# ImIntheMiddle/VATL4Pose-WACV2024

Measured on AMD Instinct MI355X. Metric: frames/sec pose-infer+uncertainty, 256x192 17-kp, higher is better.
Workload: dtype f32; 1 GPU; SimpleBaseline-R50 256x192 inference + decode + local-peak + THC-L1, 1024-frame synthetic video per GPU; frames_per_gpu=1024, batch=1024, tracks=4, parallelism=frame-sharded x1

## Files before the change

### include/vatl_hip.h

```cpp
#ifndef VATL_HIP_H
#define VATL_HIP_H

#include <stdint.h>

#ifdef __cplusplus
extern "C" {
#endif

#define VATL_VERSION 100
#define VATL_EINVAL  (-1)
#define VATL_ELAUNCH (-2)

int         vatl_version(void);
const char* vatl_last_error(void);

int vatl_flop_meter_begin(void);
int vatl_flop_meter_end(double* direct_flops, double* winograd_flops, int64_t* direct_launches, int64_t* winograd_launches);
#define VATL_ROUTE_NAMES "igemm,igemm_bnbwd,igemm_dma,persistent_1x1,streamk,rows_1x1,bottleneck_chain,stem_pool,halo_3x3," \
                         "winograd,winograd_2h,winograd_bnbwd,winograd_persist,winograd_c32,wgrad,winograd_wgrad,winograd_wgrad_2h," \
                         "winograd_wgrad_table,winograd_f4,winograd_f4_bnbwd,gemm1x1_ring,winograd_deconv43"
int vatl_flop_meter_routes(int64_t* counts, int n);


int vatl_nchw_to_nhwc(const float* src, float* dst, int N, int C, int H, int W, int Cpad, void* stream);
int vatl_nhwc_to_nchw(const float* src, float* dst, int N, int C, int H, int W, void* stream);

int vatl_pack_conv_weight(const float* w_oihw, float* w_packed, int Cout, int Cin, int R, int S,
                          int CoutPad, int Spad, int CinPad, void* stream);
int vatl_pack_deconv4x4s2_weight(const float* w_iohw, float* w_packed, int Cin, int Cout, int CoutPad, void* stream);
int64_t vatl_stem_pool_weight_floats(void);
int vatl_pack_stem_pool_weight(const float* w_oihw, float* packed, void* stream);
int vatl_stem_pool_supported(int H, int W);
int vatl_stem7x7s2_pool_fwd(const float* x_nchw, const float* w_packed, const float* scale, const float* bias, float* y_nhwc,
                            int N, int H, int W, void* stream);
int64_t vatl_stem3_weight_floats(void);
// ... 230 lines not shown
int vatl_conv3x3_winograd_fwd(const float* x, const float* u, const float* scale, const float* bias, const float* residual, float* y,
                              int N, int H, int W, int Cin, int Cout, int relu, void* stream);
int vatl_winograd_last_route(void);
int64_t vatl_winograd_stats_row_blocks(int64_t N, int H, int W);
int vatl_conv3x3_winograd_fwd_stats(const float* x, const float* u, float* y, double* stats, int64_t* row_blocks_used, int N, int H, int W,
                                    int Cin, int Cout, void* stream);
int64_t vatl_winograd_deconv_weight_floats(int Cout, int Cin);
int vatl_pack_winograd_deconv_weight(const float* w, float* u, int Cout, int Cin, void* stream);
int vatl_deconv4x4s2_winograd_fwd(const float* x, const float* u, const float* scale, const float* bias, float* y, int N, int H, int W,
                                  int Cin, int Cout, int relu, void* stream);
int64_t vatl_winograd_deconv43_weight_floats(int Cout, int Cin);
int vatl_pack_winograd_deconv43_weight(const float* w, float* u, int Cout, int Cin, void* stream);
int vatl_deconv4x4s2_winograd43_supported(int N, int H, int W, int Cin, int Cout);
int vatl_deconv4x4s2_winograd43_fwd(const float* x, const float* u, const float* scale, const float* bias, float* y, int N, int H, int W,
                                    int Cin, int Cout, int relu, void* stream);
int64_t vatl_winograd_deconv_stats_row_blocks(int64_t N, int H, int W);
int vatl_deconv4x4s2_winograd_fwd_stats(const float* x, const float* u, float* y, double* stats, int64_t* row_blocks_used, int N, int H, int W,
                                        int Cin, int Cout, void* stream);
int64_t vatl_conv3x3_winograd_wgrad_workspace_floats(int Cout, int Cin, int64_t N, int H, int W);
int vatl_conv3x3_winograd_wgrad(const float* x, const float* dz, float* dw, float* workspace, int N, int H, int W, int Cin, int Cout, void* stream);
int64_t vatl_deconv4x4s2_winograd_wgrad_workspace_floats(int Cin, int Cout, int64_t N, int H, int W);
int vatl_deconv4x4s2_winograd_wgrad(const float* x, const float* dy, float* dw, float* workspace, int N, int H, int W, int Cin, int Cout,
                                    void* stream);
int64_t vatl_winograd_deconv_dgrad_weight_floats(int Cin, int Cout);
int vatl_pack_winograd_deconv_dgrad_weight(const float* w, float* u, int Cin, int Cout, void* stream);
int vatl_deconv4x4s2_winograd_dgrad(const float* dz, const float* u, const float* residual, float* dx, int N, int H, int W, int Cin, int Cout,
                                    void* stream);
int vatl_deconv4x4s2_winograd_dgrad_bnbwd(const float* dz, const float* u, const float* residual, float* dx, int N, int H, int W, int Cin,
                                          int Cout, const float* bn_z, const float* bn_mask_y, const float* bn_scale, const float* bn_bias,
                                          const float* bn_mean, const float* bn_invstd, double* stats, int64_t* row_blocks_used, void* stream);
// ... 12 lines not shown
```

### vatl4pose-wacv2024_amd/alphapose/models/hip_engine.py

```python
from __future__ import annotations

import time
import weakref

import torch
import torch.nn as nn

import vatl_hip as vh

MAX_CHUNK = 1024



WINOGRAD = True
ROWS_GEMM = True
ROWS_GEMM_K = (128, 256)
WINO_C32 = True
WINO_F4 = True
DECONV_43 = True


class _Conv:
    __slots__ = ("w", "u", "u32", "u4", "wsrc", "wino", "c32", "f4", "scale", "bias", "cout", "r", "s", "stride", "pad")

    def __init__(self, conv: nn.Conv2d, bn: nn.BatchNorm2d | None):
        assert conv.groups == 1 and conv.dilation == (1, 1)
        assert conv.stride[0] == conv.stride[1] and conv.padding[0] == conv.padding[1]
        self.w = vh.pack_conv_weight(conv.weight.detach())
        self.cout, _, self.r, self.s = conv.weight.shape
        self.stride, self.pad = conv.stride[0], conv.padding[0]
        self.u = self.u32 = self.u4 = None
        self.wino = WINOGRAD and (self.r, self.s, self.stride, self.pad) == (3, 3, 1, 1) and conv.in_channels % 16 == 0 and self.cout % 4 == 0
        self.c32 = self.wino and WINO_C32 and conv.in_channels == 32 and self.cout == 32
        self.f4 = self.wino and WINO_F4 and conv.in_channels >= 64 and conv.in_channels % 16 == 0 and self.cout % 64 == 0
        self.wsrc = conv.weight.detach() if self.wino else None
        cb = conv.bias.detach() if conv.bias is not None else None
        if bn is not None:
            self.scale, self.bias = vh.bn_fold(_d(bn.weight), _d(bn.bias), bn.running_mean, bn.running_var, bn.eps, cb)
        elif cb is not None:
            self.scale, self.bias = vh.bn_fold(None, None, None, None, 0.0, cb, channels=self.cout)
        else:
            self.scale = self.bias = None

    def __call__(self, x, relu, residual=None, out_nchw=False, out=None):
        if self.wino and not out_nchw and not vh.latency_mode():
            if self.c32 and vh.conv3x3_winograd_c32_supported(x.shape[0], x.shape[1], x.shape[2], 32, 32):
                if self.u32 is None:
                    self.u32 = vh.pack_winograd_c32_weight(self.wsrc)
                return vh.conv3x3_winograd_c32_fwd(x, self.u32, self.scale, self.bias, relu, residual=residual, out=out)
            if self.f4 and vh.conv3x3_winograd_f4_supported(x.shape[0], x.shape[1], x.shape[2], x.shape[3], self.cout):
                if self.u4 is None:
                    self.u4 = vh.pack_winograd_f4_weight(self.wsrc)
                return vh.conv3x3_winograd_f4_fwd(x, self.u4, self.scale, self.bias, self.cout, relu, residual=residual, out=out)
            if self.u is None:
                self.u = vh.pack_winograd_weight(self.wsrc)
            return vh.conv3x3_winograd_fwd(x, self.u, self.scale, self.bias, self.cout, relu, residual=residual, out=out)
        if (ROWS_GEMM and self.r == 1 and self.stride == 1 and not out_nchw and not vh.latency_mode() and x.shape[-1] in ROWS_GEMM_K
                and vh.conv1x1_rows_supported(x.shape[-1], 0, self.cout, x.shape[0] * x.shape[1] * x.shape[2])):
            return vh.conv1x1_rows_fwd(x, self.w, self.scale, self.bias, self.cout, relu, residual=residual, out=out)
        return vh.conv2d_fwd(x, self.w, self.scale, self.bias, self.cout, self.r, self.s, self.stride, self.pad, relu,
                             residual=residual, out_nchw=out_nchw, out=out)


class _Deconv:
    __slots__ = ("w", "u", "u43", "wsrc", "d43", "scale", "bias", "cout")

    def __init__(self, dc: nn.ConvTranspose2d, bn: nn.BatchNorm2d):
        assert dc.kernel_size == (4, 4) and dc.stride == (2, 2) and dc.padding == (1, 1) and dc.bias is None
        self.cout = dc.weight.shape[1]
        self.u = self.u43 = None
        self.d43 = WINOGRAD and DECONV_43 and dc.weight.shape[0] % 16 == 0 and self.cout % 64 == 0
        self.wsrc = dc.weight.detach() if self.d43 else None
        if WINOGRAD and dc.weight.shape[0] % 16 == 0 and self.cout % 4 == 0:
            self.u = vh.pack_winograd_deconv_weight(dc.weight.detach())
        self.w = vh.pack_deconv_weight(dc.weight.detach())
        self.scale, self.bias = vh.bn_fold(_d(bn.weight), _d(bn.bias), bn.running_mean, bn.running_var, bn.eps)
# ... 498 lines not shown
```

### vatl4pose-wacv2024_amd/csrc/common.h

```cpp
#pragma once
#include <hip/hip_runtime.h>
#include <atomic>
#include <cstdarg>
#include <cstdio>
#include <cstdint>

#include "vatl_hip.h"

namespace vatl {

char* err_buf();
int fail(int code, const char* fmt, ...);

void meter_add(int kind, double flops);
enum MeterRoute {
    kRouteIgemm = 0, kRouteIgemmBnBwd, kRouteIgemmDma, kRoutePersistent1x1, kRouteStreamK, kRouteRows, kRouteChain, kRouteStemPool, kRouteHalo,
    kRouteWino, kRouteWino2H, kRouteWinoBnBwd, kRouteWinoPersist, kRouteWinoC32, kRouteWgrad, kRouteWinoWgrad, kRouteWinoWgrad2H,
    kRouteWinoWgradTable, kRouteWinoF4, kRouteWinoF4BnBwd, kRouteGemm1x1Ring, kRouteWinoDeconv43, kRouteCount
};
void meter_route(int route);

inline int check_launch(const char* what) {
    hipError_t e = hipGetLastError();
    if (e != hipSuccess) return fail(VATL_ELAUNCH, "%s: %s", what, hipGetErrorString(e));
    return 0;
}

inline int ensure_dynamic_lds(const void* kern, int bytes, std::atomic<unsigned>& done_mask, const char* what) {
    int d = 0;
    if (hipGetDevice(&d) != hipSuccess) return fail(VATL_ELAUNCH, "%s: no current device", what);
    const unsigned bit = 1u << (d & 31);
    if (done_mask.load(std::memory_order_acquire) & bit) return 0;
    hipError_t e = hipFuncSetAttribute(kern, hipFuncAttributeMaxDynamicSharedMemorySize, bytes);
// ... 59 lines not shown
```

### vatl4pose-wacv2024_amd/csrc/pack.hip

```cpp
#include "glue_common.h"
#include "winograd_pack.h"

namespace vatl {

template <class I>
__device__ __forceinline__ float pack_conv_elem(const float* __restrict__ w, I i, int Cout, int Cin, int R, int S, int Spad, int CinPad) {
    const I c = i % (I)CinPad;
    I t = i / (I)CinPad;
    const I s = t % (I)Spad; t /= (I)Spad;
    const I r = t % (I)R;
    const I o = t / (I)R;
    float v = 0.f;
    if ((int)o < Cout && (int)s < S && (int)c < Cin) v = w[(((long long)o * Cin + c) * R + r) * S + s];
    return v;
}

template <class I>
__device__ __forceinline__ float pack_deconv_elem(const float* __restrict__ w, I i, int Cin, int Cout, int CoutPad) {
    const I c = i % (I)Cin;
    I t = i / (I)Cin;
    const int tx = (int)(t & 1); t >>= 1;
    const int ty = (int)(t & 1); t >>= 1;
    const I o = t % (I)CoutPad;
    const int ph = (int)(t / (I)CoutPad);
// ... 66 lines not shown
    if (c >= C) return;
    float s = 1.f, b = 0.f;
    if (var) {
        s = (gamma ? gamma[c] : 1.f) / sqrtf(var[c] + eps);
        b = (beta ? beta[c] : 0.f) - mean[c] * s;
    }
    if (cbias) b += cbias[c] * s;
    scale[c] = s;
    bias[c] = b;
}

__global__ __launch_bounds__(256) void wino43_pack_kernel(const float* __restrict__ w, float* __restrict__ out, int Cout, int Cin) {
    wino43_pack_block(w, out, Cout, Cin, blockIdx.x, threadIdx.x);
}

__global__ __launch_bounds__(256) void pack_multi_kernel(const VatlPackJob* __restrict__ jobs, int njobs) {
    __shared__ int sj;
    if (threadIdx.x == 0) {
        int lo = 0, hi = njobs - 1;
        const long long b = blockIdx.x;
        while (lo < hi) {
            const int mid = (lo + hi + 1) >> 1;
            if (jobs[mid].first_block <= b) lo = mid; else hi = mid - 1;
        }
        sj = lo;
    }
    __syncthreads();
    const VatlPackJob* J = jobs + sj;
    const float* __restrict__ w = J->src;
    float* __restrict__ out = J->dst;
// ... 47 lines not shown
    hipLaunchKernelGGL(pack_deconv_weight_kernel, dim3(ew_grid(16LL * CoutPad * Cin)), dim3(256), 0, (hipStream_t)stream, w, out, Cin, Cout, CoutPad);
    return check_launch("pack_deconv4x4s2_weight");
}

extern "C" int64_t vatl_winograd_deconv43_weight_floats(int Cout, int Cin) { return 4LL * 20 * Cout * Cin; }

extern "C" int vatl_pack_winograd_deconv43_weight(const float* w, float* u, int Cout, int Cin, void* stream) {
    if (!w || !u || Cout <= 0 || Cin <= 0) return fail(VATL_EINVAL, "pack_winograd_deconv43_weight: null pointer or empty filter");
    if (Cin % 16 != 0 || Cout % 64 != 0) return fail(VATL_EINVAL, "pack_winograd_deconv43_weight: Cin %d must be a multiple of 16 and Cout %d of 64", Cin, Cout);
    const long long blocks = 4LL * (Cout / 32) * (Cin / 8);
    if (blocks > 0x7FFFFFFF) return fail(VATL_EINVAL, "pack_winograd_deconv43_weight: filter too large");
    hipLaunchKernelGGL(wino43_pack_kernel, dim3((unsigned)blocks), dim3(256), 0, (hipStream_t)stream, w, u, Cout, Cin);
    return check_launch("wino43_pack");
}

extern "C" int vatl_pack_dgrad_weight(const float* w_oihw, float* out, int Cout, int Cin, int R, int S, int CinPad, int CoutK,
                                      int ntaps, const int* tap_r, const int* tap_s, void* stream) {
    if (!w_oihw || !out || !tap_r || !tap_s || ntaps < 1 || ntaps > 16 || CinPad < Cin || CoutK < Cout) return fail(VATL_EINVAL, "pack_dgrad_weight: bad arguments");
    TapList t{};
    t.n = ntaps;
    for (int i = 0; i < ntaps; ++i) {
        if (tap_r[i] < 0 || tap_r[i] >= R || tap_s[i] < 0 || tap_s[i] >= S) return fail(VATL_EINVAL, "pack_dgrad_weight: tap %d out of range", i);
        t.r[i] = tap_r[i]; t.s[i] = tap_s[i];
    }
    hipLaunchKernelGGL(pack_dgrad_weight_kernel, dim3((unsigned)((long long)cdiv(CinPad, 32) * ntaps * cdiv(CoutK, 32))), dim3(256), 0, (hipStream_t)stream,
                       w_oihw, out, Cout, Cin, R, S, CinPad, CoutK, t);
    return check_launch("pack_dgrad_weight");
}

extern "C" int vatl_pack_weights_multi(const VatlPackJob* jobs_device, int njobs, int64_t total_blocks, void* stream) {
// ... 13 lines not shown
```

### vatl4pose-wacv2024_amd/csrc/winograd_pack.h

```cpp
#pragma once

namespace vatl {

__device__ __forceinline__ void wino_pack_block(const float* __restrict__ w, float* __restrict__ out, int mode, int w_i, int Cout, int Cin, int NH,
                                                long long bl, int tid) {
    const int steps = Cin >> 3;
    int phase = 0;
    if (mode >= 2) {
        const long long per = (long long)((Cout + 32 * NH - 1) / (32 * NH)) * NH * steps;
        phase = (int)(bl / per);
        bl -= phase * per;
        out += phase * per * 4096;
    }
    const int n32 = (int)(bl / steps), step = (int)(bl - (long long)n32 * steps);
    const int nl = tid & 31, cc = tid >> 5;
    const int n = n32 * 32 + nl, c = step * 8 + cc;
    const int n_tile = n32 / NH, nh = n32 - n_tile * NH;
    const int lane = (cc >> 2) * 32 + nl, tt = cc & 3;
    double tg[4][3];
    if (mode >= 2) {
        const int py = phase >> 1, px = phase & 1;
        double g[2][2];
#pragma unroll
        for (int a = 0; a < 2; ++a)
// ... 59 lines not shown
        for (int b = 0; b < 2; ++b) g[a][b] = (double)w[(((long long)c * Cout + n) * 4 + (3 - py - 2 * a)) * 4 + (3 - px - 2 * b)];
    float* o = out + ((((long long)((n32 >> 1) * steps + step) * 20) * 2 + (n32 & 1)) * 64 + (cc >> 2) * 32 + nl) * 4 + (cc & 3);
#pragma unroll
    for (int xi = 0; xi < 5; ++xi)
#pragma unroll
        for (int nu = 0; nu < 4; ++nu) {
            double v = 0.0;
#pragma unroll
            for (int a = 0; a < 2; ++a)
#pragma unroll
                for (int b = 0; b < 2; ++b) v += G4[xi][a] * g[a][b] * G3[nu][b];
            o[(long long)(xi * 4 + nu) * 512] = (float)v;
        }
}

__device__ __forceinline__ void f4_pack_item(const float* __restrict__ w, float* __restrict__ u, int dgrad, int w_i, int Cout, int Cin, long long id) {
    const int nbg = Cout >> 4;
    const long long total = (long long)(Cin >> 4) * 36 * nbg * 64;
    if (id >= total) return;
    const int lane = (int)(id & 63);
    const int blk = (int)((id >> 6) % nbg);
    const int pos = (int)((id >> 6) / nbg % 36);
    const int stage = (int)((id >> 6) / nbg / 36);
    const int xi = pos / 6, nu = pos - 6 * xi;
    const double G[6][3] = {{0.25, 0, 0}, {-1.0 / 6, -1.0 / 6, -1.0 / 6}, {-1.0 / 6, 1.0 / 6, -1.0 / 6}, {1.0 / 24, 1.0 / 12, 1.0 / 6}, {1.0 / 24, -1.0 / 12, 1.0 / 6}, {0, 0, 1}};
    const int n = 16 * blk + (lane & 15);
    float o[4];
#pragma unroll
    for (int s = 0; s < 4; ++s) {
        const int c = 16 * stage + 4 * (lane >> 4) + s;
// ... 14 lines not shown
```

### vatl4pose-wacv2024_amd/vatl_hip/__init__.py

```python
from __future__ import annotations

import ctypes as C
import os
import threading as _threading

import torch

_HERE = os.path.dirname(os.path.abspath(__file__))
LIB_PATH = os.environ.get("VATL_HIP_LIB") or os.path.join(_HERE, "libvatl_hip.so")

_p = C.c_void_p
_i = C.c_int
_f = C.c_float
_d = C.c_double
_i64 = C.c_int64

SIGNATURES = {
    "vatl_version": (_i, []),
    "vatl_last_error": (C.c_char_p, []),
    "vatl_flop_meter_begin": (_i, []),
    "vatl_flop_meter_end": (_i, [_p, _p, _p, _p]),
    "vatl_flop_meter_routes": (_i, [_p, _i]),
    "vatl_nchw_to_nhwc": (_i, [_p, _p, _i, _i, _i, _i, _i, _p]),
    "vatl_nhwc_to_nchw": (_i, [_p, _p, _i, _i, _i, _i, _p]),
# ... 77 lines not shown
    "vatl_conv3x3_winograd_wgrad_workspace_floats": (_i64, [_i, _i, _i64, _i, _i]),
    "vatl_conv3x3_winograd_wgrad": (_i, [_p] * 4 + [_i] * 5 + [_p]),
    "vatl_deconv4x4s2_winograd_wgrad_workspace_floats": (_i64, [_i, _i, _i64, _i, _i]),
    "vatl_deconv4x4s2_winograd_wgrad": (_i, [_p] * 4 + [_i] * 5 + [_p]),
    "vatl_winograd_deconv_dgrad_weight_floats": (_i64, [_i, _i]),
    "vatl_pack_winograd_deconv_dgrad_weight": (_i, [_p, _p, _i, _i, _p]),
    "vatl_deconv4x4s2_winograd_dgrad": (_i, [_p] * 4 + [_i] * 5 + [_p]),
    "vatl_deconv4x4s2_winograd_dgrad_bnbwd": (_i, [_p] * 4 + [_i] * 5 + [_p] * 9),
    "vatl_winograd_deconv_weight_floats": (_i64, [_i, _i]),
    "vatl_pack_winograd_deconv_weight": (_i, [_p, _p, _i, _i, _p]),
    "vatl_deconv4x4s2_winograd_fwd": (_i, [_p] * 5 + [_i] * 6 + [_p]),
    "vatl_winograd_deconv43_weight_floats": (_i64, [_i, _i]),
    "vatl_pack_winograd_deconv43_weight": (_i, [_p, _p, _i, _i, _p]),
    "vatl_deconv4x4s2_winograd43_supported": (_i, [_i, _i, _i, _i, _i]),
    "vatl_deconv4x4s2_winograd43_fwd": (_i, [_p] * 5 + [_i] * 6 + [_p]),
    "vatl_winograd_deconv_stats_row_blocks": (_i64, [_i64, _i, _i]),
    "vatl_deconv4x4s2_winograd_fwd_stats": (_i, [_p, _p, _p, _p, _p, _i, _i, _i, _i, _i, _p]),
    "vatl_conv2d_fwd_stats": (_i, [_p, _p, _p, _p, _p, _i, _i, _i, _i, _i, _i, _i, _i, _i, _i, _p]),
    "vatl_deconv4x4s2_fwd_stats": (_i, [_p, _p, _p, _p, _p, _i, _i, _i, _i, _i, _i, _p]),
    "vatl_bn_train_finalize": (_i, [_p, _i64, _i64, _i, _p, _p, _p, _p, _f, _f, _p, _p, _p, _p, _p]),
    "vatl_maxpool3x3s2_bwd": (_i, [_p, _p, _p, _i, _i, _i, _i, _p]),
    "vatl_maxpool3x3s2_fwd_idx": (_i, [_p, _p, _p, _i, _i, _i, _i, _p]),
    "vatl_pack_weights_multi": (_i, [_p, _i, _i64, _p]),
    "vatl_adamw_multi_block_elems": (_i64, []),
    "vatl_checksum_block_words": (_i64, []),
    "vatl_checksum_multi": (_i, [_p, _i, _i64, _p, _p]),
    "vatl_maxpool3x3s2_fwd_idx_affine": (_i, [_p, _p, _p, _p, _p, _i, _i, _i, _i, _p]),
    "vatl_bn_train_bwd_relu_pool": (_i, [_p, _p, _p, _p, _p, _p, _p, _p, _p, _p, _p, _i, _i, _i, _i, _p, _p, _p]),
    "vatl_maxpool3x3s2_bwd_idx": (_i, [_p, _p, _p, _i, _i, _i, _i, _p]),
    "vatl_pixelunshuffle2": (_i, [_p, _p, _i, _i, _i, _i, _p]),
# ... 98 lines not shown
    y = torch.empty((n, h, w, cpad), device=x.device, dtype=torch.float32)
    _check(lib().vatl_nchw_to_nhwc(_ptr(x), _ptr(y), n, c, h, w, cpad, _stream()), "vatl_nchw_to_nhwc")
    return y


def nhwc_to_nchw(x: torch.Tensor) -> torch.Tensor:
    n, h, w, c = x.shape
    y = torch.empty((n, c, h, w), device=x.device, dtype=torch.float32)
    _check(lib().vatl_nhwc_to_nchw(_ptr(x), _ptr(y), n, c, h, w, _stream()), "vatl_nhwc_to_nchw")
    return y



ROUTE_NAMES = ("igemm", "igemm_bnbwd", "igemm_dma", "persistent_1x1", "streamk", "rows_1x1", "bottleneck_chain", "stem_pool", "halo_3x3", "winograd",
               "winograd_2h", "winograd_bnbwd", "winograd_persist", "winograd_c32", "wgrad", "winograd_wgrad", "winograd_wgrad_2h", "winograd_wgrad_table", "winograd_f4", "winograd_f4_bnbwd",
               "gemm1x1_ring", "winograd_deconv43")


class flop_meter:

    def __enter__(self):
        _check(lib().vatl_flop_meter_begin(), "flop_meter_begin")
        self.direct = self.winograd = self.total = 0.0
        self.direct_launches = self.winograd_launches = 0
        return self

    @staticmethod
    def launches_now() -> int:
        counts = (C.c_int64 * len(ROUTE_NAMES))()
        _check(min(0, lib().vatl_flop_meter_routes(counts, len(ROUTE_NAMES))), "flop_meter_routes")
        return int(sum(counts))
# ... 264 lines not shown
    if tuple(w.shape[2:]) != (4, 4):
        raise VatlError("pack_winograd_deconv_weight: 4x4 filters only")
    return _pack(("winograd_deconv", w.data_ptr(), tuple(w.shape)), w, lambda: (
        int(lib().vatl_winograd_deconv_weight_floats(cout, cin)), "vatl_pack_winograd_deconv_weight", (cout, cin),
        _winograd_fields(_PACK_WINOGRAD_DECONV, cout, cin, 4, cout)))


def pack_winograd_deconv43_weight(w: torch.Tensor) -> torch.Tensor:
    cin, cout = w.shape[:2]
    if tuple(w.shape[2:]) != (4, 4):
        raise VatlError("pack_winograd_deconv43_weight: 4x4 filters only")
    return _pack(("winograd_deconv43", w.data_ptr(), tuple(w.shape)), w, lambda: (
        int(lib().vatl_winograd_deconv43_weight_floats(cout, cin)), "vatl_pack_winograd_deconv43_weight", (cout, cin), None), planned=False)


def pack_winograd_deconv_dgrad_weight(w: torch.Tensor) -> torch.Tensor:
    cin, cout = w.shape[:2]
    if tuple(w.shape[2:]) != (4, 4):
        raise VatlError("pack_winograd_deconv_dgrad_weight: 4x4 filters only")
    return _pack(("winograd_deconv_dgrad", w.data_ptr(), tuple(w.shape)), w, lambda: (
        int(lib().vatl_winograd_deconv_dgrad_weight_floats(cin, cout)), "vatl_pack_winograd_deconv_dgrad_weight", (cin, cout),
        _winograd_fields(_PACK_WINOGRAD_DECONV_DGRAD, cin, cout, 4, cout)))


def pack_conv1x1_dual_weight(w1, scale1, bias1, w2, scale2, bias2):
    cout, c1 = w1.shape[:2]
    c2 = w2.shape[1]
    cpad = conv_cout_pad(cout)
    out = torch.empty((cpad, c1 + c2), device=w1.device, dtype=torch.float32)
    bias = torch.empty(cout, device=w1.device, dtype=torch.float32)
# ... 26 lines not shown
    out = torch.empty(int(lib().vatl_stem3_weight_floats()), device=w.device, dtype=torch.float32)
    _check(lib().vatl_pack_stem3_weight(_ptr(w), _ptr(out), _stream()), "vatl_pack_stem3_weight")
    return out


def bn_fold(gamma, beta, mean, var, eps: float, conv_bias=None, channels: int | None = None):
    c = channels if channels is not None else (var.numel() if var is not None else conv_bias.numel())
    dev = (var if var is not None else conv_bias).device
    scale = torch.empty(c, device=dev, dtype=torch.float32)
    bias = torch.empty(c, device=dev, dtype=torch.float32)
    _check(lib().vatl_bn_fold(_ptr(gamma), _ptr(beta), _ptr(mean), _ptr(var), _ptr(conv_bias), eps, _ptr(scale), _ptr(bias), c, _stream()), "vatl_bn_fold")
    return scale, bias



def conv2d_fwd(x, w_packed, scale, bias, cout: int, r: int, s: int, stride: int, pad: int, relu: bool,
               residual=None, out_nchw: bool = False, out=None):
    n, h, w, cin = x.shape
    ho = (h + 2 * pad - r) // stride + 1
    wo = (w + 2 * pad - s) // stride + 1
    shape = (n, cout, ho, wo) if out_nchw else (n, ho, wo, cout)
    y = out if out is not None else torch.empty(shape, device=x.device, dtype=torch.float32)
    _check(lib().vatl_conv2d_fwd(_ptr(x), _ptr(w_packed), _ptr(scale), _ptr(bias), _ptr(residual), _ptr(y), n, h, w, cin, cout,
                                 w_packed.shape[0], r, s, stride, pad, int(relu), int(out_nchw), _stream()), "vatl_conv2d_fwd")
    return y


def conv1x1_dual_fwd(a, x, w_packed, bias, cout: int, stride2: int, relu: bool, out=None):
    n, ho, wo, c1 = a.shape
    _, h2, w2, c2 = x.shape
    y = out if out is not None else torch.empty((n, ho, wo, cout), device=a.device, dtype=torch.float32)
    _check(lib().vatl_conv1x1_dual_fwd(_ptr(a), _ptr(x), _ptr(w_packed), _ptr(bias), _ptr(y), n, ho, wo, c1, h2, w2, c2, stride2, cout,
                                       w_packed.shape[0], int(relu), _stream()), "vatl_conv1x1_dual_fwd")
    return y


def conv1x1_rows_supported(k1: int, k2: int, n: int, m: int) -> bool:
# ... 879 lines not shown
```

Measured before the change: 17030 frames/s.

## Add polyphase Winograd F(4x4? ,3x3) kernel for stride-2 3x3 convolutions

Adds a new Winograd kernel for stride-2 3x3 convs. It splits the filter into four polyphase sub-filters (2x2 taps) and transforms each into a Winograd domain, producing 4x3 output tiles, with matching weight packing and buffer-load-to-LDS staging into MFMA accumulation. The ResNet-50 downsampling convs in layers 2-4 are routed to it when there is no residual, the output is NHWC, and the shape meets H%8 and W%6. This cuts multiply work compared with the direct implicit GEMM. In exchange it adds transform overhead and fp32 rounding differences, and it only applies to shapes that meet the divisibility constraints.

```diff
diff --git a/include/vatl_hip.h b/include/vatl_hip.h
--- a/include/vatl_hip.h
+++ b/include/vatl_hip.h
@@ -18,7 +18,7 @@
 int vatl_flop_meter_end(double* direct_flops, double* winograd_flops, int64_t* direct_launches, int64_t* winograd_launches);
 #define VATL_ROUTE_NAMES "igemm,igemm_bnbwd,igemm_dma,persistent_1x1,streamk,rows_1x1,bottleneck_chain,stem_pool,halo_3x3," \
                          "winograd,winograd_2h,winograd_bnbwd,winograd_persist,winograd_c32,wgrad,winograd_wgrad,winograd_wgrad_2h," \
-                         "winograd_wgrad_table,winograd_f4,winograd_f4_bnbwd,gemm1x1_ring,winograd_deconv43"
+                         "winograd_wgrad_table,winograd_f4,winograd_f4_bnbwd,gemm1x1_ring,winograd_deconv43,winograd_s2_43"
 int vatl_flop_meter_routes(int64_t* counts, int n);
 
 
@@ -279,6 +279,11 @@
 int vatl_deconv4x4s2_winograd43_supported(int N, int H, int W, int Cin, int Cout);
 int vatl_deconv4x4s2_winograd43_fwd(const float* x, const float* u, const float* scale, const float* bias, float* y, int N, int H, int W,
                                     int Cin, int Cout, int relu, void* stream);
+int64_t vatl_winograd_s2_43_weight_floats(int Cout, int Cin);
+int vatl_pack_winograd_s2_43_weight(const float* w, float* u, int Cout, int Cin, void* stream);
+int vatl_conv3x3s2_winograd43_supported(int N, int H, int W, int Cin, int Cout);
+int vatl_conv3x3s2_winograd43_fwd(const float* x, const float* u, const float* scale, const float* bias, float* y, int N, int H, int W,
+                                  int Cin, int Cout, int relu, void* stream);
 int64_t vatl_winograd_deconv_stats_row_blocks(int64_t N, int H, int W);
 int vatl_deconv4x4s2_winograd_fwd_stats(const float* x, const float* u, float* y, double* stats, int64_t* row_blocks_used, int N, int H, int W,
                                         int Cin, int Cout, void* stream);
diff --git a/vatl4pose-wacv2024_amd/alphapose/models/hip_engine.py b/vatl4pose-wacv2024_amd/alphapose/models/hip_engine.py
--- a/vatl4pose-wacv2024_amd/alphapose/models/hip_engine.py
+++ b/vatl4pose-wacv2024_amd/alphapose/models/hip_engine.py
@@ -18,10 +18,11 @@
 WINO_C32 = True
 WINO_F4 = True
 DECONV_43 = True
+S2_43 = True
 
 
 class _Conv:
-    __slots__ = ("w", "u", "u32", "u4", "wsrc", "wino", "c32", "f4", "scale", "bias", "cout", "r", "s", "stride", "pad")
+    __slots__ = ("w", "u", "u32", "u4", "us2", "wsrc", "wino", "c32", "f4", "s2", "scale", "bias", "cout", "r", "s", "stride", "pad")
 
     def __init__(self, conv: nn.Conv2d, bn: nn.BatchNorm2d | None):
         assert conv.groups == 1 and conv.dilation == (1, 1)
@@ -33,7 +34,9 @@
         self.wino = WINOGRAD and (self.r, self.s, self.stride, self.pad) == (3, 3, 1, 1) and conv.in_channels % 16 == 0 and self.cout % 4 == 0
         self.c32 = self.wino and WINO_C32 and conv.in_channels == 32 and self.cout == 32
         self.f4 = self.wino and WINO_F4 and conv.in_channels >= 64 and conv.in_channels % 16 == 0 and self.cout % 64 == 0
-        self.wsrc = conv.weight.detach() if self.wino else None
+        self.us2 = None
+        self.s2 = WINOGRAD and S2_43 and (self.r, self.s, self.stride, self.pad) == (3, 3, 2, 1) and conv.in_channels % 16 == 0 and self.cout % 64 == 0
+        self.wsrc = conv.weight.detach() if self.wino or self.s2 else None
         cb = conv.bias.detach() if conv.bias is not None else None
         if bn is not None:
             self.scale, self.bias = vh.bn_fold(_d(bn.weight), _d(bn.bias), bn.running_mean, bn.running_var, bn.eps, cb)
@@ -58,8 +61,13 @@
         if (ROWS_GEMM and self.r == 1 and self.stride == 1 and not out_nchw and not vh.latency_mode() and x.shape[-1] in ROWS_GEMM_K
                 and vh.conv1x1_rows_supported(x.shape[-1], 0, self.cout, x.shape[0] * x.shape[1] * x.shape[2])):
             return vh.conv1x1_rows_fwd(x, self.w, self.scale, self.bias, self.cout, relu, residual=residual, out=out)
+        us2 = None
+        if self.s2 and residual is None and not out_nchw and not vh.latency_mode():
+            if self.us2 is None and vh.conv3x3s2_winograd43_supported(x.shape[0], x.shape[1], x.shape[2], x.shape[3], self.cout):
+                self.us2 = vh.pack_winograd_s2_43_weight(self.wsrc)
+            us2 = self.us2
         return vh.conv2d_fwd(x, self.w, self.scale, self.bias, self.cout, self.r, self.s, self.stride, self.pad, relu,
-                             residual=residual, out_nchw=out_nchw, out=out)
+                             residual=residual, out_nchw=out_nchw, out=out, u_s2=us2)
 
 
 class _Deconv:
diff --git a/vatl4pose-wacv2024_amd/csrc/common.h b/vatl4pose-wacv2024_amd/csrc/common.h
--- a/vatl4pose-wacv2024_amd/csrc/common.h
+++ b/vatl4pose-wacv2024_amd/csrc/common.h
@@ -16,7 +16,7 @@
 enum MeterRoute {
     kRouteIgemm = 0, kRouteIgemmBnBwd, kRouteIgemmDma, kRoutePersistent1x1, kRouteStreamK, kRouteRows, kRouteChain, kRouteStemPool, kRouteHalo,
     kRouteWino, kRouteWino2H, kRouteWinoBnBwd, kRouteWinoPersist, kRouteWinoC32, kRouteWgrad, kRouteWinoWgrad, kRouteWinoWgrad2H,
-    kRouteWinoWgradTable, kRouteWinoF4, kRouteWinoF4BnBwd, kRouteGemm1x1Ring, kRouteWinoDeconv43, kRouteCount
+    kRouteWinoWgradTable, kRouteWinoF4, kRouteWinoF4BnBwd, kRouteGemm1x1Ring, kRouteWinoDeconv43, kRouteWinoS2_43, kRouteCount
 };
 void meter_route(int route);
 
diff --git a/vatl4pose-wacv2024_amd/csrc/pack.hip b/vatl4pose-wacv2024_amd/csrc/pack.hip
--- a/vatl4pose-wacv2024_amd/csrc/pack.hip
+++ b/vatl4pose-wacv2024_amd/csrc/pack.hip
@@ -104,6 +104,10 @@
     wino43_pack_block(w, out, Cout, Cin, blockIdx.x, threadIdx.x);
 }
 
+__global__ __launch_bounds__(256) void wino_s2_43_pack_kernel(const float* __restrict__ w, float* __restrict__ out, int Cout, int Cin) {
+    wino_s2_43_pack_block(w, out, Cout, Cin, blockIdx.x, threadIdx.x);
+}
+
 __global__ __launch_bounds__(256) void pack_multi_kernel(const VatlPackJob* __restrict__ jobs, int njobs) {
     __shared__ int sj;
     if (threadIdx.x == 0) {
@@ -181,6 +185,17 @@
     return check_launch("wino43_pack");
 }
 
+extern "C" int64_t vatl_winograd_s2_43_weight_floats(int Cout, int Cin) { return 72LL * Cout * Cin; }
+
+extern "C" int vatl_pack_winograd_s2_43_weight(const float* w, float* u, int Cout, int Cin, void* stream) {
+    if (!w || !u || Cout <= 0 || Cin <= 0) return fail(VATL_EINVAL, "pack_winograd_s2_43_weight: null pointer or empty filter");
+    if (Cin % 16 != 0 || Cout % 64 != 0) return fail(VATL_EINVAL, "pack_winograd_s2_43_weight: Cin %d must be a multiple of 16 and Cout %d of 64", Cin, Cout);
+    const long long blocks = 4LL * (Cout / 32) * (Cin / 8);
+    if (blocks > 0x7FFFFFFF) return fail(VATL_EINVAL, "pack_winograd_s2_43_weight: filter too large");
+    hipLaunchKernelGGL(wino_s2_43_pack_kernel, dim3((unsigned)blocks), dim3(256), 0, (hipStream_t)stream, w, u, Cout, Cin);
+    return check_launch("wino_s2_43_pack");
+}
+
 extern "C" int vatl_pack_dgrad_weight(const float* w_oihw, float* out, int Cout, int Cin, int R, int S, int CinPad, int CoutK,
                                       int ntaps, const int* tap_r, const int* tap_s, void* stream) {
     if (!w_oihw || !out || !tap_r || !tap_s || ntaps < 1 || ntaps > 16 || CinPad < Cin || CoutK < Cout) return fail(VATL_EINVAL, "pack_dgrad_weight: bad arguments");
diff --git a/vatl4pose-wacv2024_amd/csrc/winograd_pack.h b/vatl4pose-wacv2024_amd/csrc/winograd_pack.h
--- a/vatl4pose-wacv2024_amd/csrc/winograd_pack.h
+++ b/vatl4pose-wacv2024_amd/csrc/winograd_pack.h
@@ -97,6 +97,41 @@
         }
 }
 
+__device__ __forceinline__ void wino_s2_43_pack_block(const float* __restrict__ w, float* __restrict__ out, int Cout, int Cin, long long bl, int tid) {
+    const int steps = Cin >> 3;
+    const long long per = (long long)(Cout >> 5) * steps;
+    const int phase = (int)(bl / per);
+    bl -= phase * per;
+    const int n32 = (int)(bl / steps), step = (int)(bl - (long long)n32 * steps);
+    const int nl = tid & 31, cc = tid >> 5;
+    const int n = n32 * 32 + nl, c = step * 8 + cc;
+    const int by = phase >> 1, bx = phase & 1;
+    const double G4[5][2] = {{0.5, 0.0}, {-0.5, -0.5}, {-1.0 / 6, 1.0 / 6}, {1.0 / 6, 1.0 / 3}, {0.0, 1.0}};
+    const double G3[4][2] = {{1.0, 0.0}, {0.5, 0.5}, {0.5, -0.5}, {0.0, -1.0}};
+    double g[2][2];
+#pragma unroll
+    for (int a = 0; a < 2; ++a)
+#pragma unroll
+        for (int b = 0; b < 2; ++b)
+            g[a][b] = (2 * a + by < 3 && 2 * b + bx < 3) ? (double)w[(((long long)n * Cin + c) * 3 + (2 * a + by)) * 3 + (2 * b + bx)] : 0.0;
+    const long long gstep = (long long)bx * steps + step;
+    float* o = out + (long long)(n32 >> 1) * steps * 36864 + (by ? (long long)steps * 20480 + gstep * 8192 : gstep * 10240) +
+               ((n32 & 1) * 64 + (cc >> 2) * 32 + nl) * 4 + (cc & 3);
+#pragma unroll
+    for (int xi = 0; xi < 5; ++xi) {
+        if (by && xi == 4) continue;
+#pragma unroll
+        for (int nu = 0; nu < 4; ++nu) {
+            double v = 0.0;
+#pragma unroll
+            for (int a = 0; a < 2; ++a)
+#pragma unroll
+                for (int b = 0; b < 2; ++b) v += G4[xi][a] * g[a][b] * G3[nu][b];
+            o[(long long)(xi * 4 + nu) * 512] = (float)v;
+        }
+    }
+}
+
 __device__ __forceinline__ void f4_pack_item(const float* __restrict__ w, float* __restrict__ u, int dgrad, int w_i, int Cout, int Cin, long long id) {
     const int nbg = Cout >> 4;
     const long long total = (long long)(Cin >> 4) * 36 * nbg * 64;
diff --git a/vatl4pose-wacv2024_amd/csrc/winograd_s2_43.hip b/vatl4pose-wacv2024_amd/csrc/winograd_s2_43.hip
--- /dev/null
+++ b/vatl4pose-wacv2024_amd/csrc/winograd_s2_43.hip
@@ -0,0 +1,313 @@
+#include "common.h"
+#include "buffer.h"
+
+#include <algorithm>
+#include <atomic>
+#include <type_traits>
+
+namespace vatl {
+
+struct S2W43Params {
+    const float* x;
+    const float* u;
+    const float* scale;
+    const float* bias;
+    float* y;
+    int N, H, W, Cin, Cout;
+    int OH, OW;
+    int TH, TW, tpi, Mtiles;
+    int m_tiles, n_tiles;
+    int relu;
+    int sp;
+    int rn;
+    unsigned x_bytes, u_bytes, y_bytes;
+    FastDivU d_TH, d_TW, d_tpi, d_grp, d_rn, d_rn_last;
+};
+
+constexpr unsigned S2W_OOB = 0xFFFF0000u;
+constexpr int S2W_TB = 32;
+constexpr int S2W_CK = 16;
+constexpr int S2W_NQ = S2W_TB + 1;
+constexpr int S2W_ROWE = 3 * S2W_NQ + 1;
+constexpr int S2W_ROWF = S2W_ROWE * S2W_CK;
+constexpr int S2W_ITEMS = 5 * S2W_ROWE * 4;
+constexpr int S2W_NDMA = (S2W_ITEMS + 63) / 64;
+constexpr int S2W_ROW4_DMA = 4 * S2W_ROWE * 4 / 64;
+constexpr int S2W_STAGE = S2W_NDMA * 256;
+constexpr int S2W_NLD = S2W_NDMA / 4;
+constexpr int S2W_LDS_BYTES = 2 * S2W_STAGE * 4;
+static_assert(S2W_NDMA % 4 == 0 && 16 * S2W_TB * 32 * 4 == S2W_LDS_BYTES, "stage buffers = output-transform tiles");
+static_assert(4 * S2W_ROWE * 4 % 64 == 0, "the fifth input row starts a DMA instruction");
+
+__device__ __forceinline__ void winograd_s2_43_body(const S2W43Params& p, float* smem) {
+    constexpr int NW = 4;
+    float* Rs = smem;
+    const int tid = threadIdx.x, lane = tid & 63, nu = __builtin_amdgcn_readfirstlane(tid >> 6);
+
+    const int bid = blockIdx.x, nblk = gridDim.x;
+    const int xcd = bid & 7, loc = bid >> 3, q8 = nblk >> 3, r8 = nblk & 7;
+    const int t = (xcd < r8 ? xcd * (q8 + 1) : r8 * (q8 + 1) + (xcd - r8) * q8) + loc;
+    const int grp = fdiv(t, p.d_grp), rem = t - grp * (p.m_tiles * p.rn);
+    const bool last_grp = p.n_tiles - grp * p.rn < p.rn;
+    const int rn_g = last_grp ? p.n_tiles - grp * p.rn : p.rn;
+    const int m_tile = fdiv(rem, last_grp ? p.d_rn_last : p.d_rn), n_tile = grp * p.rn + (rem - m_tile * rn_g);
+    const int m0 = m_tile * S2W_TB, n0 = n_tile * 64;
+
+    const __amdgpu_buffer_rsrc_t xr = buf_rsrc(p.x, p.x_bytes);
+    const __amdgpu_buffer_rsrc_t ur = buf_rsrc(p.u, p.u_bytes);
+
+    const int steps = p.sp * 2;
+    const int gsteps = 4 * steps, gsteps5 = 2 * steps;
+    const unsigned ubase = (unsigned)n_tile * (unsigned)steps * 147456u + ((unsigned)((nu * 2) * 64 + lane) << 4);
+    auto u_load = [&](auto np, f32x4 (&dst)[5], int gstep_, int half) {
+        constexpr int NP = decltype(np)::value;
+        const int g = min(gstep_, gsteps - 1);
+        const unsigned soff = g < gsteps5 ? (unsigned)g * 40960u : (unsigned)gsteps5 * 40960u + (unsigned)(g - gsteps5) * 32768u;
+        const unsigned off = ubase + (unsigned)half * 1024u + soff;
+#pragma unroll
+        for (int xi = 0; xi < NP; ++xi) dst[xi] = buf_load4(ur, off + xi * 8192u);
+    };
+    f32x4 ua[5], ub[5];
+    u_load(std::integral_constant<int, 5>{}, ua, 0, 0);
+
+    unsigned goff[S2W_NLD];
+    auto set_goff = [&](int pad_y, int pad_x) {
+        int m0 = m_tile * S2W_TB, ln = lane;
+        asm volatile("" : "+s"(m0), "+v"(ln));
+#pragma unroll
+        for (int u = 0; u < S2W_NLD; ++u) {
+            __builtin_amdgcn_sched_barrier(0);
+            const int pz = (nu + NW * u) * 64 + ln;
+            goff[u] = S2W_OOB;
+            if (pz >= S2W_ITEMS) continue;
+            const int cpos = pz & 3, e = pz >> 2;
+            const int i = e / S2W_ROWE, re = e - i * S2W_ROWE;
+            const int r = re / S2W_NQ, q = re - r * S2W_NQ;
+            if (r >= 3) continue;
+            const int chunk = cpos ^ ((q >> 2) & 3);
+            int m = m0 + q;
+            int gr = fdiv(m, p.d_TW), tx = m - gr * p.TW;
+            int xx = 3 * tx + r - pad_x;
+            if (m >= p.Mtiles || (tx == 0 && xx < 0)) {
+                m -= 1;
+                if (m < 0) continue;
+                gr = fdiv(m, p.d_TW); tx = m - gr * p.TW;
+                xx = 3 * tx + 3 + r - pad_x;
+            }
+            const int b = fdiv(gr, p.d_TH), ty = gr - b * p.TH;
+            const int yy = 4 * ty - pad_y + i;
+            if (m < p.Mtiles && (unsigned)yy < (unsigned)p.OH && (unsigned)xx < (unsigned)p.OW)
+                goff[u] = (unsigned)(((b * p.H + 2 * yy + pad_y) * p.W + 2 * xx + pad_x) * p.Cin + chunk * 4) << 2;
+        }
+    };
+    auto stage_dma = [&](int buf, int st, bool rows5) {
+        unsigned so = (unsigned)st * (S2W_CK * 4);
+        asm volatile("" : "+s"(so));
+#pragma unroll
+        for (int u = 0; u < S2W_NLD; ++u) {
+            if (!rows5 && nu + NW * u >= S2W_ROW4_DMA) continue;
+            __builtin_amdgcn_raw_ptr_buffer_load_lds(xr, (lds_void*)(Rs + buf * S2W_STAGE + (nu + NW * u) * 256), 16,
+                                                     goff[u] + so, 0, 0, 0);
+        }
+    };
+    set_goff(1, 1);
+    stage_dma(0, 0, true);
+
+    const int ja = nu == 0 ? 0 : (nu == 2 ? 2 : 1);
+    const int jb = nu == 0 ? 2 : (nu == 1 ? 2 : (nu == 2 ? 1 : 3));
+    const float sgn = nu == 1 ? 1.f : -1.f;
+    int ca, cb;
+    auto set_cols = [&](int pad_x) {
+        int ln = lane;
+        asm volatile("" : "+v"(ln));
+        const int tl = ln & 31, h = ln >> 5;
+        const int m = min(m0 + tl, p.Mtiles - 1);
+        const int gr = fdiv(m, p.d_TW), tx = m - gr * p.TW;
+        auto col = [&](int j) {
+            const int xx = 3 * tx + j - pad_x;
+            const int q = tl + j / 3;
+            return (unsigned)xx < (unsigned)p.OW ? ((j % 3) * S2W_NQ + q) * S2W_CK + ((h ^ ((q >> 2) & 3)) << 2) : 3 * S2W_NQ * S2W_CK + (h << 2);
+        };
+        ca = col(ja); cb = col(jb);
+    };
+
+    f32x16 accs[2][5];
+#pragma unroll
+    for (int hh = 0; hh < 2; ++hh)
+#pragma unroll
+        for (int xi = 0; xi < 5; ++xi)
+#pragma unroll
+            for (int e = 0; e < 16; ++e) accs[hh][xi][e] = 0.f;
+
+    asm volatile("s_waitcnt vmcnt(0)" ::: "memory");
+    __syncthreads();
+
+    auto make_v = [&](auto np, f32x4 (&v)[5], const float* Rb, int x8) {
+        constexpr int NP = decltype(np)::value;
+        f32x4 tc[NP];
+#pragma unroll
+        for (int i = 0; i < NP; ++i) {
+            const f32x4 da = *reinterpret_cast<const f32x4*>(Rb + i * S2W_ROWF + (ca ^ x8));
+            const f32x4 db = *reinterpret_cast<const f32x4*>(Rb + i * S2W_ROWF + (cb ^ x8));
+            tc[i] = da + sgn * db;
+        }
+        const f32x4 s = tc[3] - tc[1];
+        v[0] = 2.f * (tc[0] - tc[2]) + s;
+        v[1] = s - (tc[1] + tc[2]);
+        v[2] = 2.f * tc[1] + (tc[3] - 3.f * tc[2]);
+        v[3] = s;
+        if constexpr (NP == 5) v[4] = (tc[4] - tc[2]) - 2.f * s;
+    };
+    auto mfma_group = [&](auto np, f32x16 (&ac)[5], const f32x4 (&v)[5], const f32x4 (&uu)[5]) {
+        constexpr int NP = decltype(np)::value;
+#pragma unroll
+        for (int tt = 0; tt < 4; ++tt)
+#pragma unroll
+            for (int xi = 0; xi < NP; ++xi)
+                ac[xi] = __builtin_amdgcn_mfma_f32_32x32x2f32(v[xi][tt], uu[xi][tt], ac[xi], 0, 0, 0);
+    };
+
+    auto run_phase = [&](auto np, int ph, int gs0) {
+        constexpr int NP = decltype(np)::value;
+        set_cols(1 - (ph & 1));
+        for (int st = 0; st < p.sp; ++st) {
+            const int gs = gs0 + st, buf = gs & 1;
+            const float* Rb = Rs + buf * S2W_STAGE;
+            const bool wrap = st + 1 == p.sp;
+            if (wrap && ph < 3) set_goff(1 - ((ph + 1) >> 1), 1 - ((ph + 1) & 1));
+            f32x4 v[5];
+            u_load(np, ub, 2 * gs, 1);
+            __builtin_amdgcn_sched_barrier(0);
+            make_v(np, v, Rb, 0);
+            mfma_group(np, accs[0], v, ua);
+            __builtin_amdgcn_sched_barrier(0);
+            u_load(np, ua, 2 * gs + 1, 0);
+            __builtin_amdgcn_sched_barrier(0);
+            mfma_group(np, accs[1], v, ub);
+            __builtin_amdgcn_sched_barrier(0);
+            u_load(np, ub, 2 * gs + 1, 1);
+            if (!(wrap && ph == 3)) stage_dma(buf ^ 1, wrap ? 0 : st + 1, wrap ? ph + 1 < 2 : ph < 2);
+            __builtin_amdgcn_sched_barrier(0);
+            make_v(np, v, Rb, 8);
+            mfma_group(np, accs[0], v, ua);
+            __builtin_amdgcn_sched_barrier(0);
+            u_load(np, ua, 2 * gs + 2, 0);
+            __builtin_amdgcn_sched_barrier(0);
+            mfma_group(np, accs[1], v, ub);
+            __builtin_amdgcn_sched_barrier(0);
+            asm volatile("s_waitcnt vmcnt(0)" ::: "memory");
+            __syncthreads();
+        }
+    };
+    run_phase(std::integral_constant<int, 5>{}, 0, 0);
+    run_phase(std::integral_constant<int, 5>{}, 1, p.sp);
+    run_phase(std::integral_constant<int, 4>{}, 2, 2 * p.sp);
+    run_phase(std::integral_constant<int, 4>{}, 3, 3 * p.sp);
+
+    const __amdgpu_buffer_rsrc_t yr = buf_rsrc(p.y, p.y_bytes);
+    const int c4 = tid & 7, tl = tid >> 3;
+    const unsigned cstep = (unsigned)p.Cout << 2, rstep = (unsigned)(p.OW * p.Cout) << 2;
+    const bool valid = m0 + tl < p.Mtiles;
+    unsigned obase;
+    {
+        const int m = min(m0 + tl, p.Mtiles - 1);
+        const int b = fdiv(m, p.d_tpi), r = m - b * p.tpi;
+        const int ty = fdiv(r, p.d_TW), tx = r - ty * p.TW;
+        obase = (unsigned)(((b * p.OH + 4 * ty) * p.OW + 3 * tx) * p.Cout + n0 + c4 * 4) << 2;
+    }
+    const float lo = p.relu ? 0.f : -INFINITY;
+    float* Ps = smem;
+#pragma unroll
+    for (int hh = 0; hh < 2; ++hh) {
+        const int n = n0 + 32 * hh + c4 * 4;
+        f32x4 sc = {1.f, 1.f, 1.f, 1.f}, bi = {0.f, 0.f, 0.f, 0.f};
+        if (p.scale) sc = *reinterpret_cast<const f32x4*>(p.scale + n);
+        if (p.bias) bi = *reinterpret_cast<const f32x4*>(p.bias + n);
+        {
+            const int cl = lane & 31;
+            f32x16 (&ac)[5] = accs[hh];
+#pragma unroll
+            for (int e = 0; e < 16; ++e) {
+                const int row = (e & 3) + 8 * (e >> 2) + 4 * (lane >> 5);
+                const float sum = ac[1][e] + ac[2][e], dif = ac[1][e] - ac[2][e], m3 = ac[3][e];
+                Ps[((nu * 4 + 0) * S2W_TB + row) * 32 + cl] = ac[0][e] + sum + m3;
+                Ps[((nu * 4 + 1) * S2W_TB + row) * 32 + cl] = dif + 2.f * m3;
+                Ps[((nu * 4 + 2) * S2W_TB + row) * 32 + cl] = sum + 4.f * m3;
+                Ps[((nu * 4 + 3) * S2W_TB + row) * 32 + cl] = dif + 8.f * m3 + ac[4][e];
+            }
+        }
+        lds_barrier();
+#pragma unroll
+        for (int a = 0; a < 4; ++a) {
+            f32x4 pq[4];
+#pragma unroll
+            for (int k = 0; k < 4; ++k) pq[k] = *reinterpret_cast<const f32x4*>(&Ps[((k * 4 + a) * S2W_TB + tl) * 32 + c4 * 4]);
+            f32x4 yv[3];
+            yv[0] = pq[0] + pq[1] + pq[2];
+            yv[1] = pq[1] - pq[2];
+            yv[2] = pq[1] + pq[2] + pq[3];
+            if (valid) {
+#pragma unroll
+                for (int b = 0; b < 3; ++b) {
+                    f32x4 o;
+#pragma unroll
+                    for (int c = 0; c < 4; ++c) o[c] = fmaxf(yv[b][c] * sc[c] + bi[c], lo);
+                    buf_store4(yr, obase + (unsigned)hh * 128u + (unsigned)a * rstep + (unsigned)b * cstep, o);
+                }
+            }
+        }
+        if (hh == 0) lds_barrier();
+    }
+}
+
+__global__ __launch_bounds__(256, 2) void winograd_s2_43_kernel(S2W43Params p) {
+    extern __shared__ __attribute__((aligned(16))) float smem[];
+    winograd_s2_43_body(p, smem);
+}
+
+static std::atomic<unsigned> g_s2w43_lds_done;
+
+static bool s2w43_in_range(long long N, int H, int W, int Cin, int Cout) {
+    const long long mt = N * (H / 8) * (W / 6), xe = N * H * W * Cin, ye = N * (H / 2) * (W / 2) * Cout, ue = 72LL * Cout * Cin;
+    return xe <= (long long)(S2W_OOB / 4) && ye < (1LL << 30) && ue < (1LL << 28) && mt < (1LL << 30) && Cin / S2W_CK < 1024 &&
+           (mt + S2W_TB - 1) / S2W_TB * (Cout / 64) < (1LL << 31);
+}
+
+}
+
+using namespace vatl;
+
+extern "C" int vatl_conv3x3s2_winograd43_supported(int N, int H, int W, int Cin, int Cout) {
+    if (N <= 0 || H <= 0 || W <= 0 || Cin <= 0 || Cout <= 0) return 0;
+    if (H % 8 != 0 || W % 6 != 0 || Cin % 16 != 0 || Cout % 64 != 0) return 0;
+    return s2w43_in_range(N, H, W, Cin, Cout) ? 1 : 0;
+}
+
+extern "C" int vatl_conv3x3s2_winograd43_fwd(const float* x, const float* u, const float* scale, const float* bias, float* y, int N, int H, int W,
+                                             int Cin, int Cout, int relu, void* stream) {
+    if (!x || !u || !y) return fail(VATL_EINVAL, "conv3x3s2_winograd43_fwd: null pointer");
+    if (!vatl_conv3x3s2_winograd43_supported(N, H, W, Cin, Cout))
+        return fail(VATL_EINVAL, "conv3x3s2_winograd43_fwd: %d x %dx%d x %d -> %d is outside H %% 8 == 0, W %% 6 == 0, Cin %% 16 == 0, Cout %% 64 == 0 and 32-bit offsets",
+                    N, H, W, Cin, Cout);
+    S2W43Params p{};
+    p.x = x; p.u = u; p.scale = scale; p.bias = bias; p.y = y;
+    p.N = N; p.H = H; p.W = W; p.Cin = Cin; p.Cout = Cout; p.relu = relu;
+    p.OH = H / 2; p.OW = W / 2;
+    p.TH = p.OH / 4; p.TW = p.OW / 3; p.tpi = p.TH * p.TW;
+    p.Mtiles = N * p.tpi;
+    p.m_tiles = cdiv(p.Mtiles, S2W_TB);
+    p.n_tiles = Cout / 64;
+    p.sp = Cin / S2W_CK;
+    p.x_bytes = (unsigned)((long long)N * H * W * Cin * 4);
+    p.y_bytes = (unsigned)((long long)N * p.OH * p.OW * Cout * 4);
+    p.u_bytes = (unsigned)(72LL * Cout * Cin * 4);
+    p.rn = std::max(1, std::min(p.n_tiles, std::max(2, 2048 / (18 * Cin))));
+    p.d_TH = make_fastdiv(p.TH); p.d_TW = make_fastdiv(p.TW); p.d_tpi = make_fastdiv(p.tpi);
+    p.d_grp = make_fastdiv((unsigned)(p.m_tiles * p.rn)); p.d_rn = make_fastdiv(p.rn);
+    p.d_rn_last = make_fastdiv(p.n_tiles % p.rn ? p.n_tiles % p.rn : p.rn);
+    if (int rc = ensure_dynamic_lds((const void*)winograd_s2_43_kernel, S2W_LDS_BYTES, g_s2w43_lds_done, "winograd_s2_43")) return rc;
+    hipLaunchKernelGGL(winograd_s2_43_kernel, dim3((unsigned)(p.m_tiles * p.n_tiles)), dim3(256), S2W_LDS_BYTES, (hipStream_t)stream, p);
+    meter_add(0, 2.0 * ((double)p.m_tiles * S2W_TB) * 72.0 * (double)Cin * (double)Cout);
+    meter_route(kRouteWinoS2_43);
+    return check_launch("winograd_s2_43");
+}
diff --git a/vatl4pose-wacv2024_amd/vatl_hip/__init__.py b/vatl4pose-wacv2024_amd/vatl_hip/__init__.py
--- a/vatl4pose-wacv2024_amd/vatl_hip/__init__.py
+++ b/vatl4pose-wacv2024_amd/vatl_hip/__init__.py
@@ -115,6 +115,10 @@
     "vatl_pack_winograd_deconv43_weight": (_i, [_p, _p, _i, _i, _p]),
     "vatl_deconv4x4s2_winograd43_supported": (_i, [_i, _i, _i, _i, _i]),
     "vatl_deconv4x4s2_winograd43_fwd": (_i, [_p] * 5 + [_i] * 6 + [_p]),
+    "vatl_winograd_s2_43_weight_floats": (_i64, [_i, _i]),
+    "vatl_pack_winograd_s2_43_weight": (_i, [_p, _p, _i, _i, _p]),
+    "vatl_conv3x3s2_winograd43_supported": (_i, [_i, _i, _i, _i, _i]),
+    "vatl_conv3x3s2_winograd43_fwd": (_i, [_p] * 5 + [_i] * 6 + [_p]),
     "vatl_winograd_deconv_stats_row_blocks": (_i64, [_i64, _i, _i]),
     "vatl_deconv4x4s2_winograd_fwd_stats": (_i, [_p, _p, _p, _p, _p, _i, _i, _i, _i, _i, _p]),
     "vatl_conv2d_fwd_stats": (_i, [_p, _p, _p, _p, _p, _i, _i, _i, _i, _i, _i, _i, _i, _i, _i, _p]),
@@ -243,7 +247,7 @@
 
 ROUTE_NAMES = ("igemm", "igemm_bnbwd", "igemm_dma", "persistent_1x1", "streamk", "rows_1x1", "bottleneck_chain", "stem_pool", "halo_3x3", "winograd",
                "winograd_2h", "winograd_bnbwd", "winograd_persist", "winograd_c32", "wgrad", "winograd_wgrad", "winograd_wgrad_2h", "winograd_wgrad_table", "winograd_f4", "winograd_f4_bnbwd",
-               "gemm1x1_ring", "winograd_deconv43")
+               "gemm1x1_ring", "winograd_deconv43", "winograd_s2_43")
 
 
 class flop_meter:
@@ -538,6 +542,14 @@
         int(lib().vatl_winograd_deconv43_weight_floats(cout, cin)), "vatl_pack_winograd_deconv43_weight", (cout, cin), None), planned=False)
 
 
+def pack_winograd_s2_43_weight(w: torch.Tensor) -> torch.Tensor:
+    cout, cin = w.shape[:2]
+    if tuple(w.shape[2:]) != (3, 3):
+        raise VatlError("pack_winograd_s2_43_weight: 3x3 filters only")
+    return _pack(("winograd_s2_43", w.data_ptr(), tuple(w.shape)), w, lambda: (
+        int(lib().vatl_winograd_s2_43_weight_floats(cout, cin)), "vatl_pack_winograd_s2_43_weight", (cout, cin), None), planned=False)
+
+
 def pack_winograd_deconv_dgrad_weight(w: torch.Tensor) -> torch.Tensor:
     cin, cout = w.shape[:2]
     if tuple(w.shape[2:]) != (4, 4):
@@ -594,13 +606,22 @@
 
 
 
+def conv3x3s2_winograd43_supported(n: int, h: int, w: int, cin: int, cout: int) -> bool:
+    return bool(lib().vatl_conv3x3s2_winograd43_supported(n, h, w, cin, cout))
+
+
 def conv2d_fwd(x, w_packed, scale, bias, cout: int, r: int, s: int, stride: int, pad: int, relu: bool,
-               residual=None, out_nchw: bool = False, out=None):
+               residual=None, out_nchw: bool = False, out=None, u_s2=None):
     n, h, w, cin = x.shape
     ho = (h + 2 * pad - r) // stride + 1
     wo = (w + 2 * pad - s) // stride + 1
     shape = (n, cout, ho, wo) if out_nchw else (n, ho, wo, cout)
     y = out if out is not None else torch.empty(shape, device=x.device, dtype=torch.float32)
+    if (u_s2 is not None and (r, s, stride, pad) == (3, 3, 2, 1) and residual is None and not out_nchw
+            and conv3x3s2_winograd43_supported(n, h, w, cin, cout)):
+        _check(lib().vatl_conv3x3s2_winograd43_fwd(_ptr(x), _ptr(u_s2), _ptr(scale), _ptr(bias), _ptr(y), n, h, w, cin, cout, int(relu), _stream()),
+               "vatl_conv3x3s2_winograd43_fwd")
+        return y
     _check(lib().vatl_conv2d_fwd(_ptr(x), _ptr(w_packed), _ptr(scale), _ptr(bias), _ptr(residual), _ptr(y), n, h, w, cin, cout,
                                  w_packed.shape[0], r, s, stride, pad, int(relu), int(out_nchw), _stream()), "vatl_conv2d_fwd")
     return y
```

Measured after the change: 17330 frames/s, median of 6. 1.02x the previous value.
